# tauzn-clock/mpsfm

Hardware: AMD Instinct MI355X
Metric: BA residual-evals/sec (LM iterations/sec alongside), 200 imgs / 150k pts prior-BA (higher is better)
Workload: dtype f64; 1 GPU; C3: 200 cameras, 150000 landmarks per rank, 749145 reprojection + 674306 log-depth blocks per rank, SoftL1/Cauchy, Ceres-default LM; parallelism=single GPU, residual_blocks_total=1423451

## Files before the change

### include/mpsfm_hip_debug.h

```cpp
#ifndef MPSFM_HIP_DEBUG_H
#define MPSFM_HIP_DEBUG_H

#include "mpsfm_hip.h"

#ifdef __cplusplus
extern "C" {
#endif

typedef struct mpsfm_plan_handle mpsfm_plan_handle;

void mpsfm_debug_set(int f);
int mpsfm_debug_set_chol_trace(long long* dev_buf);
int mpsfm_debug_panel_factor(const double* dx, int waves, double* out, int* ok);

mpsfm_plan_handle* mpsfm_debug_plan_create(const uint8_t* adj, int32_t n, int32_t depth, int32_t pinv_max_tiles, int32_t inv_rows);
void mpsfm_debug_plan_destroy(mpsfm_plan_handle* h);
int64_t mpsfm_debug_plan_get(const mpsfm_plan_handle* h, int32_t what, int32_t* out, int64_t cap);

int64_t mpsfm_debug_host_cache(int64_t bytes, int32_t count);
int64_t mpsfm_debug_run_parts(int32_t nparts, int32_t reps);
int mpsfm_debug_graph_union(const uint8_t* adj, int32_t world, int32_t n, uint8_t* out);

int mpsfm_debug_pt_handoff(mpsfm_ba_handle* h);
int mpsfm_debug_direct_front(mpsfm_ba_handle* h);
int mpsfm_debug_direct_assemble(mpsfm_ba_handle* h, double radius, double* A_parent, double* A_direct, double* damp, uint8_t* live, int64_t info[4]);
int mpsfm_debug_dense_solve_given(mpsfm_ba_handle* h, const double* S, const double* rhs, int32_t n, int32_t* failed);
int mpsfm_debug_read_trace(mpsfm_ba_handle* h, long long* out, int64_t count);
int64_t mpsfm_debug_table(mpsfm_ba_handle* h, int32_t which, void* out, int64_t cap);
int64_t mpsfm_debug_host_build(const mpsfm_ba_problem* P, int32_t which, void* out, int64_t cap);
int mpsfm_debug_local_clocks(mpsfm_ba_handle* h, int64_t out[12]);
int mpsfm_debug_local_skew(int32_t chunk, int32_t phase_mask, int64_t ticks);
typedef struct mpsfm_debug_lm_ctl {
  double radius, decrease_factor, x_norm, cur_cost, fixed_cost, initial_cost;
  double last_x_cost, last_cand, last_rel, last_step_norm, last_mcc;
  int32_t term, iter, invalid_run, check_gradient, accepted, n_success, n_unsuccess, n_cost_evals, n_jac_evals, last_chol_fail, trace_len, pad_;
  double trace_cost[MPSFM_MAX_TRACE], trace_radius[MPSFM_MAX_TRACE];
  uint8_t trace_accepted[MPSFM_MAX_TRACE];
} mpsfm_debug_lm_ctl;
typedef struct mpsfm_debug_lm_opts {
  double function_tolerance, gradient_tolerance, parameter_tolerance, min_relative_decrease, max_radius, min_radius;
  int32_t max_iterations, max_invalid_steps;
} mpsfm_debug_lm_opts;
int mpsfm_debug_lm_decide(int32_t form, const mpsfm_debug_lm_ctl* ctl_in, const mpsfm_debug_lm_opts* opts, double* scal, const double* redsc, const double* part,
// ... 8 lines not shown
```

### mpsfm_amd/abi.py

```python

from __future__ import annotations

import ctypes as C
import os

MAX_TRACE = 64
INT_MAX_IRLS = 16

TERMINATION_NAMES = {
    0: "function_tolerance",
    1: "gradient_tolerance",
    2: "parameter_tolerance",
    3: "max_iterations",
    4: "min_radius",
    5: "invalid_steps",
    6: "no_variables",
}

ALLREDUCE_FN = C.CFUNCTYPE(C.c_int, C.c_void_p, C.POINTER(C.c_double), C.c_int64, C.c_int, C.c_void_p)


class CProblem(C.Structure):
    _c_name_ = "mpsfm_ba_problem"
    _fields_ = [
# ... 428 lines not shown
    "mpsfm_debug_set": (None, [C.c_int]),
    "mpsfm_debug_set_chol_trace": (C.c_int, [P]),
    "mpsfm_debug_panel_factor": (C.c_int, [P, C.c_int, P, C.POINTER(C.c_int)]),
    "mpsfm_debug_plan_create": (P, [P, I32, I32, I32, I32]),
    "mpsfm_debug_plan_destroy": (None, [P]),
    "mpsfm_debug_plan_get": (I64, [P, I32, P, I64]),
    "mpsfm_debug_host_cache": (I64, [I64, I32]),
    "mpsfm_debug_run_parts": (I64, [I32, I32]),
    "mpsfm_debug_graph_union": (C.c_int, [P, I32, I32, P]),
    "mpsfm_debug_pt_handoff": (C.c_int, [P]),
    "mpsfm_debug_direct_front": (C.c_int, [P]),
    "mpsfm_debug_direct_assemble": (C.c_int, [P, C.c_double, P, P, P, P, P]),
    "mpsfm_debug_dense_solve_given": (C.c_int, [P, P, P, I32, C.POINTER(I32)]),
    "mpsfm_debug_read_trace": (C.c_int, [P, P, I64]),
    "mpsfm_debug_table": (I64, [P, I32, P, I64]),
    "mpsfm_debug_host_build": (I64, [P, I32, P, I64]),
    "mpsfm_debug_local_clocks": (C.c_int, [P, P]),
    "mpsfm_debug_local_skew": (C.c_int, [I32, I32, I64]),
    "mpsfm_debug_lm_decide": (C.c_int, [I32, P, P, P, P, P, P, I64, I32, P, P, P]),
    "mpsfm_debug_resources": (C.c_int, [I32, P]),
}


LIB_PATH = os.path.join(os.path.dirname(os.path.abspath(__file__)), "libmpsfm_hip.so")

_lib = None


class MpsfmHipError(RuntimeError):
    def __init__(self, code: int, msg: str):
# ... 21 lines not shown
```

### mpsfm_amd/build.py

```python

from __future__ import annotations

import os
import subprocess
import sys

HERE = os.path.dirname(os.path.abspath(__file__))
CSRC = os.path.join(HERE, "csrc")
LIB = os.path.join(HERE, "libmpsfm_hip.so")
SOURCES = ["ba_kernels.hip", "sweep_dense.hip", "local_lm.hip", "build_dev.hip", "build_host.hip", "dense_chol.hip", "dev_resources.hip", "ba_comm.hip", "ba_build.hip", "ba_solver.hip", "ba_debug.hip", "tri_kernels.hip", "int_kernels.hip", "prior_kernels.hip", "triangulator.hip", "chol_plan.hip", "depth_consistency.hip", "abs_pose.hip", "rel_pose.hip", "two_view.hip", "two_view_batch.hip", "registration.hip", "dense_matches.hip", "descriptor_matches.hip", "descriptor_matches_batch.hip", "retrieval.hip", "reciprocal_matches.hip", "warp_matches.hip", "mono_priors.hip", "corr_graph.hip"]
HEADERS = ["common.h", "dev_resources.h", "ba_launch.h", "ba_handle.h", "devbuild.h", "build_host.h", "host_parts.h", "sweep_common.h", "sweep_dense_body.h", "sweep_update_body.h", "dense_tile.h", "lm_decide.h", "local_lm.h", "tri_math.h", "bilinear_sample.h", "abs_pose_math.h", "rel_pose_math.h", "rel_pose_problem.h", "two_view_math.h", "two_view_problem.h", "chol_plan.h", "call_scope.h", "lo_ransac.h", "point_grid.h", "resize_taps.h", "sim_tile.h", "sim_top2.h", "sim_topk.h", os.path.join("..", "..", "include", "mpsfm_hip.h"),
           os.path.join("..", "..", "include", "mpsfm_hip_debug.h")]


def _hipcc() -> str:
    for c in (os.environ.get("HIPCC"), "/opt/rocm/bin/hipcc", "hipcc"):
        if c and (os.path.isabs(c) and os.path.exists(c) or not os.path.isabs(c)):
            return c
    return "hipcc"


FLAGS_STAMP = os.path.join(HERE, "build", "extra_flags.txt")


def _flags_changed() -> bool:
# ... 52 lines not shown
```

### mpsfm_amd/capi.py

```python

from __future__ import annotations

import ctypes as C

import numpy as np

from .abi import (
    ALLREDUCE_FN, LIB_PATH, SIGNATURES, CAbsPoseOptions, CAbsPoseResult, CCorrGraphInfo, CDcImage, CDebugLmCtl, CDebugLmOpts, CDcSummary, CDepthGather, CDepthPriorConf,
    CDepthPriorOutput, CDepthPriorProblem, CInitCandidates, CInitPair, CIntProblem, CIntSummary, CMatchBatchReport, CMatchInfo, CMatchOptions, CNmsInfo,
    CNormalPriorConf, CNormalPriorOutput, CNormalPriorProblem, COptions, CPriorSummary, CProblem, CRansacOptions, CRecipInfo,
    CRecipOptions, CRegImage, CRelPoseOptions, CRetrievalInfo, CRetrievalOptions, CRelPoseResult, CState, CSummary, CTracks, CTriCandidates, CTwoViewBatchReport, CTwoViewLeg, CTwoViewOptions,
    CTwoViewResult, CWarpInfo, CWarpOptions, MpsfmHipError, lib,
)
from .problem import BAProblem, Tracks

EXPORTS = list(SIGNATURES)
_MATCH_DESC_ARGS = SIGNATURES["mpsfm_match_descriptors"][1]
_MATCH_MAP_ARGS = SIGNATURES["mpsfm_match_map_descriptors"][1]
_SIMPLE_NMS_ARGS = SIGNATURES["mpsfm_simple_nms"][1]
_KPIDS_ARGS = SIGNATURES["mpsfm_kpids_to_matches0"][1]
_WARP_ARGS = SIGNATURES["mpsfm_warp_matches"][1]


def _check(rc: int):
# ... 117 lines not shown

    def pt_handoff(self) -> bool:
        return bool(lib().mpsfm_debug_pt_handoff(self._h))

    def direct_front(self) -> bool:
        return bool(lib().mpsfm_debug_direct_front(self._h))

    def direct_assemble(self, radius: float = 1e4) -> dict:
        nt = self.dense_plan()["tile_columns"]
        ntiles = (nt + 1) * (nt + 2) // 2
        ap, ad = np.zeros((ntiles, 32, 32)), np.zeros((ntiles, 32, 32))
        damp, live, info = np.zeros(32 * nt), np.zeros(ntiles, np.uint8), np.zeros(4, np.int64)
        _check(lib().mpsfm_debug_direct_assemble(self._h, float(radius), ap.ctypes.data, ad.ctypes.data, damp.ctypes.data, live.ctypes.data, info.ctypes.data))
        assert int(info[0]) == nt
        return dict(parent=ap, direct=ad, damp=damp, live=live.astype(bool), nt=nt, n=int(info[1]), n_live=int(info[2]), unzeroed=int(info[3]))

    def sweep_once(self, radius: float = 1e4) -> float:
        ms = C.c_float(0)
        _check(lib().mpsfm_ba_sweep_once(self._h, radius, C.byref(ms)))
        return ms.value

    def sweep_parts(self) -> dict:
        ms, info = (C.c_float * 3)(), (C.c_int64 * 4)()
        _check(lib().mpsfm_ba_sweep_parts(self._h, ms, info))
        return dict(dense_ms=ms[0], reduce_ms=ms[1], general_ms=ms[2], dense_chunks=int(info[0]), general_chunks=int(info[1]),
                    long_tracks=int(info[2]), reduce_parts=int(info[3]))

    def dense_solve_once(self) -> float:
        ms = C.c_float(0)
        _check(lib().mpsfm_ba_dense_solve_once(self._h, C.byref(ms)))
# ... 1108 lines not shown
```

### mpsfm_amd/csrc/ba_debug.hip

```cpp
#include <algorithm>
#include <atomic>
#include <cstring>
#include <limits>
#include <vector>

#include "../../include/mpsfm_hip_debug.h"
#include "ba_handle.h"

using namespace mpsfm;

static void dense_plan_numbers(int ncv, int nt, const CholPlan& P, const DenseOverlap& ov, const LevelPlanDev& lp, double* work, int64_t sblk, int64_t v[10]) {
  const bool level = dense_level(&ov, &lp);
  const bool pinv = level && dense_pinv(work, nt, &ov, &lp) != nullptr;
  const int64_t w[10] = {ncv, nt, level ? P.nlevels : nt, P.nd_depth, pinv ? 1 : 0, (int64_t)P.items.size(), P.products, P.roles, sblk,
                         pinv ? 1 : (level ? P.nlevels : (nt + 3) / 4 + 1)};
  for (int i = 0; i < 10; ++i) v[i] = w[i];
}

extern "C" int64_t mpsfm_debug_host_cache(int64_t bytes, int32_t count) {
  std::vector<mpsfm::HostBuf<uint8_t>> first((size_t)count), second((size_t)count);
  std::vector<const void*> seen;
  for (auto& b : first) { b.alloc((size_t)bytes); b[0] = 1; b[(size_t)bytes - 1] = 2; seen.push_back(b.data()); }
  first.clear();
  int64_t reused = 0;
// ... 152 lines not shown
  MPSFM_TRY(hipMemcpyAsync(A_direct, h->d_A, sizeof(double) * img.size(), hipMemcpyDeviceToHost, s));
  MPSFM_TRY(hipMemcpyAsync(pinv.data(), a.zero_P, sizeof(double) * pinv.size(), hipMemcpyDeviceToHost, s));
  MPSFM_TRY(hipMemcpyAsync(y.data(), h->d_yc, sizeof(double) * (size_t)h->n_user, hipMemcpyDeviceToHost, s));
  MPSFM_TRY(hipMemcpyAsync(dcol.data(), h->d_diag_col, sizeof(double) * dcol.size(), hipMemcpyDeviceToHost, s));
  MPSFM_TRY(hipStreamSynchronize(s));
  MPSFM_TRY(hipGetLastError());
  h->last_radius = radius;
  const int32_t* slot_of_col = h->plan.slot_of_col.empty() ? nullptr : h->plan.slot_of_col.data();
  for (int g = 0; g < nt * 32; ++g)
    damp[g] = vec_index(slot_of_col, g, h->n) < 0 ? -1.0 : std::min(std::max(dcol[(size_t)g], h->opt.min_lm_diagonal), h->opt.max_lm_diagonal) / radius;
  int64_t bad = 0;
  for (double v : pinv) bad += v == 0.0 ? 0 : 1;
  for (int i = 0; i < h->n_user; ++i) bad += y[(size_t)i] == 0.0 ? 0 : 1;
  info[0] = nt; info[1] = h->n; info[2] = (int64_t)h->plan.asm_tiles.size(); info[3] = bad;
  return 0;
}

int mpsfm_ba_sweep_once(mpsfm_ba_handle* h, double radius, float* elapsed_ms) {
  if (!h) return fail(MPSFM_EINVAL, "handle is NULL");
  MPSFM_TRY(hipSetDevice(h->device));
  if (!h->scales_ready) if (int rc = prepare_scales(h)) return rc;
  MPSFM_TRY(hipMemsetAsync(h->d_red, 0, sizeof(double) * (size_t)h->red_count, h->stream));
  SweepArgs a = sweep_args(h, radius);
  MPSFM_TRY(hipEventRecord(h->ev[0], h->stream));
  launch_track_sweep_dense(a, h->n_dense, h->stream);
  MPSFM_TRY(hipEventRecord(h->ev[1], h->stream));
  launch_reduce_slabs(h->d_red_dests, h->n_red_dests, h->d_red_srcs, h->d_slab, h->d_Sblk, h->d_gc, h->d_wv, h->d_diagU, nullptr, h->stream);
  MPSFM_TRY(hipEventRecord(h->ev[2], h->stream));
  a.chunk0 = h->n_dense;
  launch_track_sweep(a, h->nchunks - h->n_dense, false, h->stream);
// ... 46 lines not shown
    case 20: src = h->d_red_srcs; bytes = 4 * h->n_red_srcs; break;
    case 21: src = h->cam_slot_h.data(); bytes = 4 * (int64_t)h->cam_slot_h.size(); host = true; break;
    case 23: src = h->d_blk_desc; bytes = 4 * h->n_blk_desc; break;
    case 24: src = h->d_blk_ent_start; bytes = 4 * h->n_blk_ent_start; break;
    case 25: src = h->d_ents; bytes = 4 * h->n_ents; break;
    case 26: src = h->d_part; bytes = 32 * (int64_t)h->nchunks; break;
    case 22: { static uint8_t flag; flag = h->built_on_device ? 1 : 0; src = &flag; bytes = 1; host = true; break; }
    case 27: src = h->d_lhdr; bytes = (int64_t)sizeof(LongHdr) * h->nlong; break;
    case 28: src = h->spat.sky_index.data(); bytes = 4 * (int64_t)h->spat.sky_index.size(); host = true; break;
    case 29: src = h->spat.sky_first.data(); bytes = 4 * (int64_t)h->spat.sky_first.size(); host = true; break;
    case 30: src = h->spat.sky_start.data(); bytes = 8 * (int64_t)h->spat.sky_start.size(); host = true; break;
    case 31: src = h->d_cmask; bytes = 48 * (int64_t)h->nc; break;
    case 32: src = h->d_cam_of_slot; bytes = 4 * (int64_t)std::max(h->ncv, 1); break;
    case 33: { static thread_local int64_t info[10]; if (int rc = mpsfm_ba_dense_plan(h, info)) return rc; src = info; bytes = 80; host = true; break; }
    case 34: src = h->last_launches; bytes = (int64_t)sizeof(h->last_launches); host = true; break;
    default: return fail(MPSFM_EINVAL, "unknown table");
  }
  if (!out || cap < bytes) return bytes;
  if (bytes == 0) return 0;
  if (host) { std::memcpy(out, src, (size_t)bytes); return bytes; }
  if (hipSetDevice(h->device) != hipSuccess) return fail(MPSFM_EHIP, "hipSetDevice failed");
  if (hipMemcpyAsync(out, src, (size_t)bytes, hipMemcpyDeviceToHost, h->stream) != hipSuccess) return fail(MPSFM_EHIP, "copy failed");
  if (hipStreamSynchronize(h->stream) != hipSuccess) return fail(MPSFM_EHIP, "sync failed");
  return bytes;
}

int64_t mpsfm_debug_host_build(const mpsfm_ba_problem* P, int32_t which, void* out, int64_t cap) {
  if (int rc = check_problem(P)) return rc;
  BuildOptions opt = BuildOptions::from_environment();
  TableBuild B;
// ... 177 lines not shown
```

### mpsfm_amd/csrc/ba_handle.h

```cpp
#pragma once
#include <cstdint>
#include <memory>
#include <vector>

#include "ba_launch.h"
#include "build_host.h"
#include "common.h"
#include "dev_resources.h"
#include "devbuild.h"

struct mpsfm_ba_handle {
  int device = 0;
  mpsfm::DeviceBlocks own;
  hipStream_t stream = nullptr;
  void* comm = nullptr;
  mpsfm::DenseOverlap ov;
  mpsfm::SPattern spat;
  mpsfm::BlockSky sky{nullptr, nullptr, nullptr, 0};
  mpsfm::CholPlan plan;
  mpsfm::LevelPlanDev lp;
  std::vector<int32_t> nat_slot;
  int n_user = 0;
  mpsfm_ba_options opt{};
  mpsfm::LossParams loss{};
// ... 73 lines not shown
int build_tables(const mpsfm_ba_problem* P, BuildOptions& opt, const SumExchange& exchange, bool sharded, int verbose, const Lap& lap, DeviceStages* dev,
                 TableBuild& out);
void level_plan_flags(const CholPlan& PL, LevelPlanDev& D);

int create_impl(const mpsfm_ba_problem* P, const mpsfm_ba_state* st, const mpsfm_ba_options* o, mpsfm_ba_handle** out);
int upload_state(mpsfm_ba_handle* h, const mpsfm_ba_state* st, bool as_initial);
void free_handle(mpsfm_ba_handle* h);

int comm_init_rank(mpsfm_ba_handle* h);
void comm_destroy(void* comm);
int allreduce_host(mpsfm_ba_handle* h, double* buf, int64_t count);
int allreduce_dev(mpsfm_ba_handle* h, double* buf, int64_t count);

SweepArgs sweep_args(mpsfm_ba_handle* h, double radius, const LmCtl* ctl = nullptr);
int prepare_scales(mpsfm_ba_handle* h);
int run_track_sweep(mpsfm_ba_handle* h, double radius, const LmCtl* ctl = nullptr, bool in_loop = false, bool adopt = false, bool handoff = false,
                    bool direct = false);
void run_assemble(mpsfm_ba_handle* h, double radius, const LmCtl* ctl = nullptr);
int run_dense(mpsfm_ba_handle* h, double radius, const LmCtl* ctl = nullptr, bool direct = false);
bool direct_front(mpsfm_ba_handle* h);
DirectAsm direct_asm(const mpsfm_ba_handle* h);
void direct_zero_args(mpsfm_ba_handle* h, SweepArgs& a);
bool chol_entry_list();

struct LocalSkew { int32_t chunk = 0, mask = 0; int64_t ticks = 0; };
extern LocalSkew g_local_skew;

}
```

### mpsfm_amd/csrc/ba_launch.h

```cpp
#pragma once
#include "common.h"
#include "local_lm.h"

namespace mpsfm {
enum LaunchFamily {
  kLfTrackSweep,
  kLfReduceSlabs,
  kLfAssemble,
  kLfCholLevel,
  kLfDenseRest,
  kLfUpdateSweep,
  kLfDecide,
  kLfScales,
  kLfOther,
  kLfCount
};
extern thread_local int64_t g_launches[kLfCount];
inline void count_launch(LaunchFamily f, int n = 1) { g_launches[f] += n; }

void launch_track_sweep(const SweepArgs&, int nchunks, bool diag_only, hipStream_t);
void launch_update_sweep(const SweepArgs&, int nchunks, hipStream_t, const CamUpdArgs* cu = nullptr);
void launch_track_sweep_dense(const SweepArgs&, int nchunks, hipStream_t);
void launch_reduce_slabs(const RedDest* dests, int ndest, const int32_t* srcs, const double* slab, double* Sblk, double* gc, double* wv, double* diagU,
                         const LmCtl* ctl, hipStream_t, const DirectAsm* direct = nullptr);
// ... 10 lines not shown
constexpr int kReduceThreads = 1024;
void launch_lm_decide(LmCtl* ctl, double* scal, const LmOpts& o, LmCtl* host_copy, hipStream_t, const double* redsc = nullptr);
void launch_zero(double* p, int64_t n, const LmCtl* ctl, hipStream_t);
void launch_lm_reduce_decide(const double* part, const double* part2, int64_t rows, LmCtl* ctl, double* scal, const LmOpts& o, LmCtl* host_copy, hipStream_t);
void launch_lm_prologue(const LmCtl* ctl, double* red, int64_t nred, int nc, int64_t np, double* q, double* t, double* camtab, double* pts, const double* q2,
                        const double* t2, const double* camtab2, const double* pts2, hipStream_t);
void launch_lm_accept(const LmCtl* ctl, int nc, int64_t np, double* q, double* t, double* camtab, double* pts, const double* q2, const double* t2,
                      const double* camtab2, const double* pts2, hipStream_t);
void launch_pts_sqnorm(int64_t np, const uint16_t* pt_kv, const double* pts, double* part, int nblocks, hipStream_t);
void launch_gmax_to_slot(double* redsc, int rank, hipStream_t);
void launch_lm_pack(const double* scal, double* sums, hipStream_t);
void launch_lm_init(LmCtl* ctl, const double* scal, const double* sums, hipStream_t);
void launch_permute_pts(int64_t np, const int32_t* perm, const double* src, double* dst, bool scatter, hipStream_t);
void launch_gmax_from_slots(const double* redsc, double* scal, hipStream_t);

extern int g_dbg_flags;
void launch_assemble(const AssembleArgs&, hipStream_t);
void launch_dense_solve(double* A, double* work, int nt, int n, double* y, int* fail, hipStream_t, DenseOverlap* ov, const LevelPlanDev* lp,
                        const LmCtl* ctl = nullptr, const DampArgs* damp = nullptr);
bool dense_level(const DenseOverlap* ov, const LevelPlanDev* lp);
int dense_plain_max_tiles();
int dense_inv_rows();
size_t dense_work_doubles(int nt);
double* dense_pinv(double* work, int nt, const DenseOverlap* ov, const LevelPlanDev* lp);

int local_lm_max_chunks(int device);
int launch_local_lm(const LocalArgs& a, hipStream_t s);

}
```

### mpsfm_amd/csrc/ba_solver.hip

```cpp
#include <algorithm>
#include <chrono>
#include <cstdio>
#include <cstdlib>
#include <cstring>
#include <vector>

#include "ba_handle.h"

namespace mpsfm {

LocalSkew g_local_skew;

SweepArgs sweep_args(mpsfm_ba_handle* h, double radius, const LmCtl* ctl) {
  SweepArgs a{};
  a.ctl = ctl;
  a.chunks = h->d_chunks; a.chunk_cams = h->d_chunk_cams; a.rec_cam = h->rt.rec_cam; a.rec_meta = h->rt.rec_meta;
  a.rec_xy = h->rt.rec_xy; a.rec_d = h->rt.rec_d; a.rec_m = h->rt.rec_m; a.rec_a = h->rt.rec_a;
  a.pt_rec_start = h->rt.pt_rec_start; a.pt_kv = h->rt.pt_kv; a.blk_desc = h->d_blk_desc; a.blk_ent_start = h->d_blk_ent_start; a.ents = h->d_ents;
  a.camtab = h->d_camtab; a.pts = h->d_pts; a.ps = h->d_ps; a.loss = h->loss;
  a.radius = radius; a.min_diag = h->opt.min_lm_diagonal; a.max_diag = h->opt.max_lm_diagonal; a.ncv = h->ncv; a.dbg = (g_dbg_flags >> 8) & 0xff;
  a.lhdr = h->d_lhdr; a.nlong = h->nlong; a.nchunks = h->nchunks; a.cam_slot = h->d_cam_slot; a.wl = h->d_wl;
  a.sky = h->sky;
  a.Sblk = h->d_Sblk; a.gc = h->d_gc; a.wv = h->d_wv; a.diagU = h->d_diagU; a.part = h->d_part; a.diagV = h->d_diagV;
  a.yc = h->d_yc; a.camtab2 = h->d_camtab2; a.pts2 = h->d_pts2; a.part2 = h->d_part2;
// ... 136 lines not shown
  sum->num_iterations = last.iter;
  sum->num_successful_steps = last.n_success;
  sum->num_unsuccessful_steps = last.n_unsuccess;
  sum->termination = last.term;
  sum->final_radius = last.radius;
  sum->trace_len = last.trace_len;
  for (int i = 0; i < last.trace_len; ++i) { sum->trace_cost[i] = last.trace_cost[i]; sum->trace_radius[i] = last.trace_radius[i]; sum->trace_accepted[i] = last.trace_accepted[i]; }
  return 0;
}

constexpr int kLocalRefused = 1;
constexpr double kSplitMinFront = 40e-6;
bool chol_entry_list() { const char* e = std::getenv("MPSFM_CHOL_ENTRY"); return e && std::strcmp(e, "list") == 0; }
static bool pt_handoff_enabled() { const char* e = std::getenv("MPSFM_PT_HANDOFF"); return !(e && std::atoi(e) == 0); }

static int solve_local(mpsfm_ba_handle* h, mpsfm_ba_summary* sum) {
  hipStream_t s = h->stream;
  const mpsfm_ba_options& o = h->opt;
  launch_cam_scales(h->nc, h->d_cam_slot, h->d_cmask, h->d_diagU, 0, h->d_cs, s);
  launch_build_camtab(h->nc, h->d_q, h->d_t, h->d_intr, h->d_intr_idx, h->d_cs, h->d_camtab, s);
  double* fixed_parts = h->d_scal + 12;
  MPSFM_TRY(hipMemsetAsync(h->d_scal, 0, sizeof(double) * U_COUNT, s));
  launch_fixed_cost(h, fixed_parts);
  if (int rc = prepare_scales(h)) return rc;
  h->h_ctl[0] = initial_ctl(o);
  MPSFM_TRY(hipMemcpyAsync(h->d_ctl, &h->h_ctl[0], sizeof(LmCtl), hipMemcpyHostToDevice, s));
  MPSFM_TRY(hipMemsetAsync(h->d_local_acc, 0, sizeof(double) * 2 * kLocalAccDoubles, s));
  MPSFM_TRY(hipMemsetAsync(h->d_local_sync, 0, sizeof(int64_t) * 16, s));
  LocalArgs la{};
  la.A = sweep_args(h, 0.0, nullptr);
  if (pt_handoff_enabled()) la.A.pt_fac = h->d_pt_fac;
  la.ctl = h->d_ctl;
  la.o = lm_opts_of(o);
  la.log = o.verbose > 0 ? h->d_local_log : nullptr;
  la.acc[0] = h->d_local_acc; la.acc[1] = h->d_local_acc + kLocalAccDoubles;
  la.part[0] = h->d_part; la.part[1] = h->d_part + (size_t)h->nchunks * 4;
  la.bar = reinterpret_cast<int32_t*>(h->d_local_sync); la.clk = reinterpret_cast<long long*>(h->d_local_sync + 1);
  la.ncv = h->ncv; la.nc = h->nc; la.nchunks = h->nchunks;
  la.q = h->d_q; la.t = h->d_t; la.camtab = h->d_camtab; la.pts = h->d_pts; la.cs = h->d_cs; la.fixed_parts = fixed_parts;
  la.skew_chunk = g_local_skew.chunk; la.skew_mask = g_local_skew.ticks > 0 ? g_local_skew.mask : 0; la.skew_ticks = g_local_skew.ticks;
  if (launch_local_lm(la, s) != (int)hipSuccess) {
    (void)hipGetLastError();
    MPSFM_TRY(hipStreamSynchronize(s));
// ... 29 lines not shown
  MPSFM_TRY(hipStreamSynchronize(s));
  const auto t_begin = clk::now();
  sum->num_residual_blocks = (int64_t)h->nblocks_global;
  sum->reduced_dim = h->n_user;
  std::fill(g_launches, g_launches + kLfCount, (int64_t)0);
  auto finish = [&](int rc) {
    std::copy(g_launches, g_launches + kLfCount, h->last_launches);
    sum->time_total_s = std::chrono::duration<double>(clk::now() - t_begin).count();
    return rc;
  };
  if (h->local_ok) {
    const int rc = solve_local(h, sum);
    if (rc != kLocalRefused) return finish(rc);
  }

  launch_cam_scales(h->nc, h->d_cam_slot, h->d_cmask, h->d_diagU, 0, h->d_cs, s);
  launch_build_camtab(h->nc, h->d_q, h->d_t, h->d_intr, h->d_intr_idx, h->d_cs, h->d_camtab, s);
  if (h->n == 0 && h->nvarpts_global == 0.0) {
    double fx[3], c3[3];
    if (int rc = cost_of_records(h, true, fx)) return rc;
    double fixed = fx[0] + fx[1];
    if (int rc = allreduce_host(h, &fixed, 1)) return rc;
    sum->fixed_cost = fixed;
    if (int rc = cost_of_records(h, false, c3)) return rc;
    double c = c3[0] + c3[1];
    if (int rc = allreduce_host(h, &c, 1)) return rc;
    sum->initial_cost = sum->final_cost = c + fixed;
    sum->termination = MPSFM_TERM_NO_VARIABLES;
    return finish(0);
  }
  MPSFM_TRY(hipMemsetAsync(h->d_scal, 0, sizeof(double) * U_COUNT, s));
  launch_fixed_cost(h, h->d_scal + 12);
  if (int rc = prepare_scales(h)) return rc;
  if (h->np > 0) MPSFM_TRY(hipMemcpyAsync(h->d_pts2, h->d_pts, sizeof(double) * 3 * h->np, hipMemcpyDeviceToDevice, s));
  MPSFM_TRY(hipMemsetAsync(h->d_yc, 0, sizeof(double) * (size_t)std::max(h->n_user, 1), s));
  MPSFM_TRY(hipMemsetAsync(h->d_gc, 0, sizeof(double) * (size_t)std::max(h->n_user, 1), s));
  launch_cam_update(h->nc, h->d_cam_slot, h->d_q, h->d_t, h->d_cs, h->d_yc, h->d_gc, h->d_q2, h->d_t2, h->d_scal, s);
  const int nb = (int)std::min<int64_t>(1024, std::max<int64_t>(1, (h->np + kThreads - 1) / kThreads));
  launch_pts_sqnorm(h->np, h->rt.pt_kv, h->d_pts, h->d_costpart, nb, s);
  launch_reduce_cols(h->d_costpart, nb, 1, 1, 0u, h->d_scal + U_XN_SQ_PTS, s);

  h->h_ctl[0] = initial_ctl(o);
  MPSFM_TRY(hipMemcpyAsync(h->d_ctl, &h->h_ctl[0], sizeof(LmCtl), hipMemcpyHostToDevice, s));
  double* sums = nullptr;
  if (sharded(h)) {
    sums = h->d_costpart;
    launch_lm_pack(h->d_scal, sums, s);
    if (int rc = allreduce_dev(h, sums, 3)) return rc;
  }
  launch_lm_init(h->d_ctl, h->d_scal, sums, s);
  const LmOpts lo = lm_opts_of(o);
  const LmCtl* ctl = h->d_ctl;
  const double no_radius = 0.0;
  const bool fuse_prologue = [] { const char* e = std::getenv("MPSFM_FUSE_PROLOGUE"); return !(e && std::atoi(e) == 0); }();
  const bool fuse_cam = [] { const char* e = std::getenv("MPSFM_FUSE_CAM"); return !(e && std::atoi(e) == 0); }();
  const bool pt_handoff = pt_handoff_enabled() && h->d_pt_fac != nullptr;
  h->ov.entry_list = chol_entry_list();
  const bool fused_prologue = fuse_prologue && h->nlong == 0 && h->n_dense > 0 && h->n_dense == h->nchunks;
  const bool direct = fused_prologue && direct_front(h);
  auto enqueue_front = [&](int it) -> int {
    hipEvent_t* ev = (it & 1) ? h->ev2 : h->ev;
    MPSFM_TRY(hipEventRecord(ev[0], s));
    if (!fused_prologue)
      launch_lm_prologue(h->d_ctl, h->d_red, h->red_count, h->nc, h->np, h->d_q, h->d_t, h->d_camtab, h->d_pts, h->d_q2, h->d_t2, h->d_camtab2, h->d_pts2, s);
    if (int rc = run_track_sweep(h, no_radius, ctl, true, fused_prologue, pt_handoff, direct)) return rc;
// ... 187 lines not shown
```

Measured before the change: 9.990 billion residual-block evals/s.

## Fuse BA solve setup into begin, diagonal-sweep and scales kernels

Replaces the chain of small setup launches, memsets, copies and reductions that run before the LM loop (camera scales, camtab build, scale preparation, point copy and norm, camera update, control init) with three kernels. A begin kernel clears buffers and the control block, a per-chunk diagonal sweep computes the Jacobi diagonals and also copies points and partial norms, and a single-block kernel finishes the camera scales, candidates and control fields. This cuts per-solve launch and host overhead. It adds a second linearization path that has to stay consistent with prepare_scales, and an env var keeps the old launch path available.

```diff
diff --git a/include/mpsfm_hip_debug.h b/include/mpsfm_hip_debug.h
--- a/include/mpsfm_hip_debug.h
+++ b/include/mpsfm_hip_debug.h
@@ -27,6 +27,7 @@
 int mpsfm_debug_dense_solve_given(mpsfm_ba_handle* h, const double* S, const double* rhs, int32_t n, int32_t* failed);
 int mpsfm_debug_read_trace(mpsfm_ba_handle* h, long long* out, int64_t count);
 int64_t mpsfm_debug_table(mpsfm_ba_handle* h, int32_t which, void* out, int64_t cap);
+int mpsfm_debug_solve_setup(mpsfm_ba_handle* h, int32_t local);
 int64_t mpsfm_debug_host_build(const mpsfm_ba_problem* P, int32_t which, void* out, int64_t cap);
 int mpsfm_debug_local_clocks(mpsfm_ba_handle* h, int64_t out[12]);
 int mpsfm_debug_local_skew(int32_t chunk, int32_t phase_mask, int64_t ticks);
diff --git a/mpsfm_amd/abi.py b/mpsfm_amd/abi.py
--- a/mpsfm_amd/abi.py
+++ b/mpsfm_amd/abi.py
@@ -466,6 +466,7 @@
     "mpsfm_debug_dense_solve_given": (C.c_int, [P, P, P, I32, C.POINTER(I32)]),
     "mpsfm_debug_read_trace": (C.c_int, [P, P, I64]),
     "mpsfm_debug_table": (I64, [P, I32, P, I64]),
+    "mpsfm_debug_solve_setup": (C.c_int, [P, I32]),
     "mpsfm_debug_host_build": (I64, [P, I32, P, I64]),
     "mpsfm_debug_local_clocks": (C.c_int, [P, P]),
     "mpsfm_debug_local_skew": (C.c_int, [I32, I32, I64]),
diff --git a/mpsfm_amd/build.py b/mpsfm_amd/build.py
--- a/mpsfm_amd/build.py
+++ b/mpsfm_amd/build.py
@@ -8,7 +8,7 @@
 HERE = os.path.dirname(os.path.abspath(__file__))
 CSRC = os.path.join(HERE, "csrc")
 LIB = os.path.join(HERE, "libmpsfm_hip.so")
-SOURCES = ["ba_kernels.hip", "sweep_dense.hip", "local_lm.hip", "build_dev.hip", "build_host.hip", "dense_chol.hip", "dev_resources.hip", "ba_comm.hip", "ba_build.hip", "ba_solver.hip", "ba_debug.hip", "tri_kernels.hip", "int_kernels.hip", "prior_kernels.hip", "triangulator.hip", "chol_plan.hip", "depth_consistency.hip", "abs_pose.hip", "rel_pose.hip", "two_view.hip", "two_view_batch.hip", "registration.hip", "dense_matches.hip", "descriptor_matches.hip", "descriptor_matches_batch.hip", "retrieval.hip", "reciprocal_matches.hip", "warp_matches.hip", "mono_priors.hip", "corr_graph.hip"]
+SOURCES = ["ba_kernels.hip", "sweep_dense.hip", "solve_setup.hip", "local_lm.hip", "build_dev.hip", "build_host.hip", "dense_chol.hip", "dev_resources.hip", "ba_comm.hip", "ba_build.hip", "ba_solver.hip", "ba_debug.hip", "tri_kernels.hip", "int_kernels.hip", "prior_kernels.hip", "triangulator.hip", "chol_plan.hip", "depth_consistency.hip", "abs_pose.hip", "rel_pose.hip", "two_view.hip", "two_view_batch.hip", "registration.hip", "dense_matches.hip", "descriptor_matches.hip", "descriptor_matches_batch.hip", "retrieval.hip", "reciprocal_matches.hip", "warp_matches.hip", "mono_priors.hip", "corr_graph.hip"]
 HEADERS = ["common.h", "dev_resources.h", "ba_launch.h", "ba_handle.h", "devbuild.h", "build_host.h", "host_parts.h", "sweep_common.h", "sweep_dense_body.h", "sweep_update_body.h", "dense_tile.h", "lm_decide.h", "local_lm.h", "tri_math.h", "bilinear_sample.h", "abs_pose_math.h", "rel_pose_math.h", "rel_pose_problem.h", "two_view_math.h", "two_view_problem.h", "chol_plan.h", "call_scope.h", "lo_ransac.h", "point_grid.h", "resize_taps.h", "sim_tile.h", "sim_top2.h", "sim_topk.h", os.path.join("..", "..", "include", "mpsfm_hip.h"),
            os.path.join("..", "..", "include", "mpsfm_hip_debug.h")]
 
diff --git a/mpsfm_amd/capi.py b/mpsfm_amd/capi.py
--- a/mpsfm_amd/capi.py
+++ b/mpsfm_amd/capi.py
@@ -155,6 +155,20 @@
         _check(lib().mpsfm_debug_direct_assemble(self._h, float(radius), ap.ctypes.data, ad.ctypes.data, damp.ctypes.data, live.ctypes.data, info.ctypes.data))
         assert int(info[0]) == nt
         return dict(parent=ap, direct=ad, damp=damp, live=live.astype(bool), nt=nt, n=int(info[1]), n_live=int(info[2]), unzeroed=int(info[3]))
+
+    def solve_setup(self, local: int = -1) -> dict:
+        rc = lib().mpsfm_debug_solve_setup(self._h, int(local))
+        if rc < 0:
+            _check(rc)
+        out = {"fused": bool(rc)}
+        for code, name, width in ((35, "cs", 6), (36, "ps", 3), (37, "camtab", 24), (38, "q2", 4), (39, "t2", 3), (40, "pts2", 3), (41, "x_norm", 0),
+                                  (42, "fixed_cost", 0)):
+            n = int(lib().mpsfm_debug_table(self._h, code, None, 0))
+            assert n >= 0 and n % 8 == 0, (code, n)
+            v = np.zeros(n // 8)
+            assert int(lib().mpsfm_debug_table(self._h, code, v.ctypes.data, n)) == n
+            out[name] = v.reshape(-1, width) if width else float(v[0])
+        return out
 
     def sweep_once(self, radius: float = 1e4) -> float:
         ms = C.c_float(0)
diff --git a/mpsfm_amd/csrc/ba_debug.hip b/mpsfm_amd/csrc/ba_debug.hip
--- a/mpsfm_amd/csrc/ba_debug.hip
+++ b/mpsfm_amd/csrc/ba_debug.hip
@@ -190,6 +190,17 @@
   for (int i = 0; i < h->n_user; ++i) bad += y[(size_t)i] == 0.0 ? 0 : 1;
   info[0] = nt; info[1] = h->n; info[2] = (int64_t)h->plan.asm_tiles.size(); info[3] = bad;
   return 0;
+}
+
+int mpsfm_debug_solve_setup(mpsfm_ba_handle* h, int32_t local) {
+  if (!h) return fail(MPSFM_EINVAL, "handle is NULL");
+  if (local > 0 && !h->local_ok) return fail(MPSFM_EUNSUPPORTED, "the handle does not take the single-launch solver");
+  MPSFM_TRY(hipSetDevice(h->device));
+  const bool fused = setup_fused(h);
+  if (int rc = setup_solve(h, local < 0 ? h->local_ok : local > 0)) return rc < 0 ? rc : -rc;
+  MPSFM_TRY(hipStreamSynchronize(h->stream));
+  MPSFM_TRY(hipGetLastError());
+  return fused ? 1 : 0;
 }
 
 int mpsfm_ba_sweep_once(mpsfm_ba_handle* h, double radius, float* elapsed_ms) {
@@ -266,6 +277,14 @@
     case 32: src = h->d_cam_of_slot; bytes = 4 * (int64_t)std::max(h->ncv, 1); break;
     case 33: { static thread_local int64_t info[10]; if (int rc = mpsfm_ba_dense_plan(h, info)) return rc; src = info; bytes = 80; host = true; break; }
     case 34: src = h->last_launches; bytes = (int64_t)sizeof(h->last_launches); host = true; break;
+    case 35: src = h->d_cs; bytes = 48 * (int64_t)h->nc; break;
+    case 36: src = h->d_ps; bytes = 24 * h->np; break;
+    case 37: src = h->d_camtab; bytes = 8 * (int64_t)kCamRec * h->nc; break;
+    case 38: src = h->d_q2; bytes = 32 * (int64_t)h->nc; break;
+    case 39: src = h->d_t2; bytes = 24 * (int64_t)h->nc; break;
+    case 40: src = h->d_pts2; bytes = 24 * h->np; break;
+    case 41: src = &h->d_ctl->x_norm; bytes = 8; break;
+    case 42: src = &h->d_ctl->fixed_cost; bytes = 8; break;
     default: return fail(MPSFM_EINVAL, "unknown table");
   }
   if (!out || cap < bytes) return bytes;
diff --git a/mpsfm_amd/csrc/ba_handle.h b/mpsfm_amd/csrc/ba_handle.h
--- a/mpsfm_amd/csrc/ba_handle.h
+++ b/mpsfm_amd/csrc/ba_handle.h
@@ -111,6 +111,8 @@
 
 SweepArgs sweep_args(mpsfm_ba_handle* h, double radius, const LmCtl* ctl = nullptr);
 int prepare_scales(mpsfm_ba_handle* h);
+int setup_solve(mpsfm_ba_handle* h, bool local);
+bool setup_fused(const mpsfm_ba_handle* h);
 int run_track_sweep(mpsfm_ba_handle* h, double radius, const LmCtl* ctl = nullptr, bool in_loop = false, bool adopt = false, bool handoff = false,
                     bool direct = false);
 void run_assemble(mpsfm_ba_handle* h, double radius, const LmCtl* ctl = nullptr);
diff --git a/mpsfm_amd/csrc/ba_launch.h b/mpsfm_amd/csrc/ba_launch.h
--- a/mpsfm_amd/csrc/ba_launch.h
+++ b/mpsfm_amd/csrc/ba_launch.h
@@ -48,6 +48,27 @@
 void launch_permute_pts(int64_t np, const int32_t* perm, const double* src, double* dst, bool scatter, hipStream_t);
 void launch_gmax_from_slots(const double* redsc, double* scal, hipStream_t);
 
+struct SetupArgs {
+  int32_t nc, n_user;
+  const int32_t* cam_slot; const double* cmask; const double* q; const double* t; const double* intr; const int32_t* intr_idx;
+  double* cs; double* camtab;
+  double* diagU; double* yc; double* gc; double* scal;
+  LmCtl* ctl; double radius0;
+  double* local_acc; int64_t n_local_acc;
+  int64_t* local_sync;
+  double* q2; double* t2;
+  const double* norm_part; int32_t n_norm_part;
+  int32_t init_ctl;
+};
+struct DiagArgs {
+  double* ps;
+  int64_t np;
+  double* norm_part;
+};
+void launch_solve_begin(const SetupArgs&, hipStream_t);
+void launch_diag_sweep(const SweepArgs&, const DiagArgs&, int nchunks, hipStream_t);
+void launch_solve_scales(const SetupArgs&, hipStream_t);
+
 extern int g_dbg_flags;
 void launch_assemble(const AssembleArgs&, hipStream_t);
 void launch_dense_solve(double* A, double* work, int nt, int n, double* y, int* fail, hipStream_t, DenseOverlap* ov, const LevelPlanDev* lp,
diff --git a/mpsfm_amd/csrc/ba_solver.hip b/mpsfm_amd/csrc/ba_solver.hip
--- a/mpsfm_amd/csrc/ba_solver.hip
+++ b/mpsfm_amd/csrc/ba_solver.hip
@@ -174,19 +174,76 @@
 bool chol_entry_list() { const char* e = std::getenv("MPSFM_CHOL_ENTRY"); return e && std::strcmp(e, "list") == 0; }
 static bool pt_handoff_enabled() { const char* e = std::getenv("MPSFM_PT_HANDOFF"); return !(e && std::atoi(e) == 0); }
 
+static int setup_launches(mpsfm_ba_handle* h, bool local) {
+  hipStream_t s = h->stream;
+  launch_cam_scales(h->nc, h->d_cam_slot, h->d_cmask, h->d_diagU, 0, h->d_cs, s);
+  launch_build_camtab(h->nc, h->d_q, h->d_t, h->d_intr, h->d_intr_idx, h->d_cs, h->d_camtab, s);
+  MPSFM_TRY(hipMemsetAsync(h->d_scal, 0, sizeof(double) * U_COUNT, s));
+  launch_fixed_cost(h, h->d_scal + 12);
+  if (int rc = prepare_scales(h)) return rc;
+  h->h_ctl[0] = initial_ctl(h->opt);
+  if (local) {
+    MPSFM_TRY(hipMemcpyAsync(h->d_ctl, &h->h_ctl[0], sizeof(LmCtl), hipMemcpyHostToDevice, s));
+    MPSFM_TRY(hipMemsetAsync(h->d_local_acc, 0, sizeof(double) * 2 * kLocalAccDoubles, s));
+    MPSFM_TRY(hipMemsetAsync(h->d_local_sync, 0, sizeof(int64_t) * 16, s));
+    return 0;
+  }
+  if (h->np > 0) MPSFM_TRY(hipMemcpyAsync(h->d_pts2, h->d_pts, sizeof(double) * 3 * h->np, hipMemcpyDeviceToDevice, s));
+  MPSFM_TRY(hipMemsetAsync(h->d_yc, 0, sizeof(double) * (size_t)std::max(h->n_user, 1), s));
+  MPSFM_TRY(hipMemsetAsync(h->d_gc, 0, sizeof(double) * (size_t)std::max(h->n_user, 1), s));
+  launch_cam_update(h->nc, h->d_cam_slot, h->d_q, h->d_t, h->d_cs, h->d_yc, h->d_gc, h->d_q2, h->d_t2, h->d_scal, s);
+  const int nb = (int)std::min<int64_t>(1024, std::max<int64_t>(1, (h->np + kThreads - 1) / kThreads));
+  launch_pts_sqnorm(h->np, h->rt.pt_kv, h->d_pts, h->d_costpart, nb, s);
+  launch_reduce_cols(h->d_costpart, nb, 1, 1, 0u, h->d_scal + U_XN_SQ_PTS, s);
+  MPSFM_TRY(hipMemcpyAsync(h->d_ctl, &h->h_ctl[0], sizeof(LmCtl), hipMemcpyHostToDevice, s));
+  double* sums = nullptr;
+  if (sharded(h)) {
+    sums = h->d_costpart;
+    launch_lm_pack(h->d_scal, sums, s);
+    if (int rc = allreduce_dev(h, sums, 3)) return rc;
+  }
+  launch_lm_init(h->d_ctl, h->d_scal, sums, s);
+  return 0;
+}
+bool setup_fused(const mpsfm_ba_handle* h) {
+  const char* e = std::getenv("MPSFM_SOLVE_SETUP");
+  if (e && std::strcmp(e, "launches") == 0) return false;
+  return h->opt.jacobi_scaling != 0 && h->nlong == 0 && h->nchunks > 0 && h->nc > 0;
+}
+int setup_solve(mpsfm_ba_handle* h, bool local) {
+  if (!setup_fused(h)) return setup_launches(h, local);
+  hipStream_t s = h->stream;
+  SetupArgs P{};
+  P.nc = h->nc; P.n_user = h->n_user;
+  P.cam_slot = h->d_cam_slot; P.cmask = h->d_cmask; P.q = h->d_q; P.t = h->d_t; P.intr = h->d_intr; P.intr_idx = h->d_intr_idx;
+  P.cs = h->d_cs; P.camtab = h->d_camtab;
+  P.diagU = h->d_diagU; P.yc = h->d_yc; P.gc = h->d_gc; P.scal = h->d_scal;
+  P.ctl = h->d_ctl; P.radius0 = h->opt.initial_trust_region_radius;
+  if (local) { P.local_acc = h->d_local_acc; P.n_local_acc = 2 * (int64_t)kLocalAccDoubles; P.local_sync = h->d_local_sync; }
+  else { P.q2 = h->d_q2; P.t2 = h->d_t2; P.norm_part = h->d_part2; P.n_norm_part = h->nchunks; P.init_ctl = sharded(h) ? 0 : 1; }
+  launch_solve_begin(P, s);
+  launch_fixed_cost(h, h->d_scal + 12);
+  const DiagArgs D{h->d_ps, h->np, local ? nullptr : h->d_part2};
+  launch_diag_sweep(sweep_args(h, 1.0), D, h->nchunks, s);
+  if (int rc = allreduce_dev(h, h->d_diagU, h->n_user)) return rc;
+  launch_solve_scales(P, s);
+  h->h_ctl[0] = initial_ctl(h->opt);
+  if (!local && sharded(h)) {
+    double* sums = h->d_costpart;
+    launch_lm_pack(h->d_scal, sums, s);
+    if (int rc = allreduce_dev(h, sums, 3)) return rc;
+    launch_lm_init(h->d_ctl, h->d_scal, sums, s);
+  }
+  MPSFM_TRY(hipGetLastError());
+  h->scales_ready = true;
+  return 0;
+}
+
 static int solve_local(mpsfm_ba_handle* h, mpsfm_ba_summary* sum) {
   hipStream_t s = h->stream;
   const mpsfm_ba_options& o = h->opt;
-  launch_cam_scales(h->nc, h->d_cam_slot, h->d_cmask, h->d_diagU, 0, h->d_cs, s);
-  launch_build_camtab(h->nc, h->d_q, h->d_t, h->d_intr, h->d_intr_idx, h->d_cs, h->d_camtab, s);
   double* fixed_parts = h->d_scal + 12;
-  MPSFM_TRY(hipMemsetAsync(h->d_scal, 0, sizeof(double) * U_COUNT, s));
-  launch_fixed_cost(h, fixed_parts);
-  if (int rc = prepare_scales(h)) return rc;
-  h->h_ctl[0] = initial_ctl(o);
-  MPSFM_TRY(hipMemcpyAsync(h->d_ctl, &h->h_ctl[0], sizeof(LmCtl), hipMemcpyHostToDevice, s));
-  MPSFM_TRY(hipMemsetAsync(h->d_local_acc, 0, sizeof(double) * 2 * kLocalAccDoubles, s));
-  MPSFM_TRY(hipMemsetAsync(h->d_local_sync, 0, sizeof(int64_t) * 16, s));
+  if (int rc = setup_solve(h, true)) return rc;
   LocalArgs la{};
   la.A = sweep_args(h, 0.0, nullptr);
   if (pt_handoff_enabled()) la.A.pt_fac = h->d_pt_fac;
@@ -246,9 +303,9 @@
     if (rc != kLocalRefused) return finish(rc);
   }
 
-  launch_cam_scales(h->nc, h->d_cam_slot, h->d_cmask, h->d_diagU, 0, h->d_cs, s);
-  launch_build_camtab(h->nc, h->d_q, h->d_t, h->d_intr, h->d_intr_idx, h->d_cs, h->d_camtab, s);
   if (h->n == 0 && h->nvarpts_global == 0.0) {
+    launch_cam_scales(h->nc, h->d_cam_slot, h->d_cmask, h->d_diagU, 0, h->d_cs, s);
+    launch_build_camtab(h->nc, h->d_q, h->d_t, h->d_intr, h->d_intr_idx, h->d_cs, h->d_camtab, s);
     double fx[3], c3[3];
     if (int rc = cost_of_records(h, true, fx)) return rc;
     double fixed = fx[0] + fx[1];
@@ -261,26 +318,8 @@
     sum->termination = MPSFM_TERM_NO_VARIABLES;
     return finish(0);
   }
-  MPSFM_TRY(hipMemsetAsync(h->d_scal, 0, sizeof(double) * U_COUNT, s));
-  launch_fixed_cost(h, h->d_scal + 12);
-  if (int rc = prepare_scales(h)) return rc;
-  if (h->np > 0) MPSFM_TRY(hipMemcpyAsync(h->d_pts2, h->d_pts, sizeof(double) * 3 * h->np, hipMemcpyDeviceToDevice, s));
-  MPSFM_TRY(hipMemsetAsync(h->d_yc, 0, sizeof(double) * (size_t)std::max(h->n_user, 1), s));
-  MPSFM_TRY(hipMemsetAsync(h->d_gc, 0, sizeof(double) * (size_t)std::max(h->n_user, 1), s));
-  launch_cam_update(h->nc, h->d_cam_slot, h->d_q, h->d_t, h->d_cs, h->d_yc, h->d_gc, h->d_q2, h->d_t2, h->d_scal, s);
-  const int nb = (int)std::min<int64_t>(1024, std::max<int64_t>(1, (h->np + kThreads - 1) / kThreads));
-  launch_pts_sqnorm(h->np, h->rt.pt_kv, h->d_pts, h->d_costpart, nb, s);
-  launch_reduce_cols(h->d_costpart, nb, 1, 1, 0u, h->d_scal + U_XN_SQ_PTS, s);
-
-  h->h_ctl[0] = initial_ctl(o);
-  MPSFM_TRY(hipMemcpyAsync(h->d_ctl, &h->h_ctl[0], sizeof(LmCtl), hipMemcpyHostToDevice, s));
-  double* sums = nullptr;
-  if (sharded(h)) {
-    sums = h->d_costpart;
-    launch_lm_pack(h->d_scal, sums, s);
-    if (int rc = allreduce_dev(h, sums, 3)) return rc;
-  }
-  launch_lm_init(h->d_ctl, h->d_scal, sums, s);
+  if (int rc = setup_solve(h, false)) return rc;
+
   const LmOpts lo = lm_opts_of(o);
   const LmCtl* ctl = h->d_ctl;
   const double no_radius = 0.0;
diff --git a/mpsfm_amd/csrc/solve_setup.hip b/mpsfm_amd/csrc/solve_setup.hip
--- /dev/null
+++ b/mpsfm_amd/csrc/solve_setup.hip
@@ -0,0 +1,191 @@
+#include "common.h"
+#include "ba_launch.h"
+#include "sweep_common.h"
+#include <algorithm>
+
+namespace mpsfm {
+
+__device__ __forceinline__ void camtab_row(const SetupArgs& P, int i, const double (&cs6)[6]) {
+  double* o = P.camtab + (size_t)i * kCamRec;
+  quat_to_R(P.q + 4 * i, o);
+  o[9] = P.t[3 * i]; o[10] = P.t[3 * i + 1]; o[11] = P.t[3 * i + 2];
+  const double* K = P.intr + 4 * P.intr_idx[i];
+  o[12] = K[0]; o[13] = K[1]; o[14] = K[2]; o[15] = K[3];
+  for (int k = 0; k < 6; ++k) { o[16 + k] = cs6[k]; P.cs[6 * i + k] = cs6[k]; }
+  o[22] = o[23] = 0.0;
+}
+
+__global__ __launch_bounds__(256) void k_solve_begin(SetupArgs P) {
+  const int64_t g0 = (int64_t)blockIdx.x * 256 + threadIdx.x, gstep = (int64_t)gridDim.x * 256;
+  for (int64_t i = g0; i < P.nc; i += gstep) {
+    const bool var = P.cam_slot[i] >= 0;
+    double cs6[6];
+#pragma unroll
+    for (int k = 0; k < 6; ++k) cs6[k] = var ? P.cmask[6 * i + k] : 0.0;
+    camtab_row(P, (int)i, cs6);
+  }
+  for (int64_t e = g0; e < P.n_user; e += gstep) { P.diagU[e] = 0.0; P.yc[e] = 0.0; P.gc[e] = 0.0; }
+  for (int64_t e = g0; e < U_COUNT; e += gstep) P.scal[e] = 0.0;
+  if (P.local_acc) {
+    for (int64_t e = g0; e < P.n_local_acc; e += gstep) P.local_acc[e] = 0.0;
+    for (int64_t e = g0; e < 16; e += gstep) P.local_sync[e] = 0;
+  }
+  if (blockIdx.x == 0) {
+    static_assert(sizeof(LmCtl) % 8 == 0, "the control block is cleared in 8-byte words");
+    unsigned long long* w = reinterpret_cast<unsigned long long*>(P.ctl);
+    for (int e = threadIdx.x; e < (int)(sizeof(LmCtl) / 8); e += 256) w[e] = 0ull;
+    __syncthreads();
+    if (threadIdx.x == 0) { P.ctl->radius = P.radius0; P.ctl->decrease_factor = 2.0; P.ctl->term = kLmRunning; P.ctl->check_gradient = 1; }
+  }
+}
+
+__device__ __forceinline__ double tree16(const double* p, bool is_max) {
+  double a[4];
+#pragma unroll
+  for (int k = 0; k < 4; ++k)
+    a[k] = is_max ? fmax(fmax(p[4 * k], p[4 * k + 1]), fmax(p[4 * k + 2], p[4 * k + 3])) : (p[4 * k] + p[4 * k + 1]) + (p[4 * k + 2] + p[4 * k + 3]);
+  return is_max ? fmax(fmax(a[0], a[1]), fmax(a[2], a[3])) : (a[0] + a[1]) + (a[2] + a[3]);
+}
+__global__ __launch_bounds__(kReduceThreads) void k_solve_scales(SetupArgs P) {
+  constexpr int kWaves = kReduceThreads / 64;
+  static_assert(kWaves == 16, "tree16 sums sixteen wave results");
+  __shared__ double s_red[4 * kWaves];
+  const double zero6[6] = {0.0, 0.0, 0.0, 0.0, 0.0, 0.0};
+  double step = 0.0, xn = 0.0, gmax = 0.0;
+  for (int i = threadIdx.x; i < P.nc; i += kReduceThreads) {
+    const int slot = P.cam_slot[i];
+    double cs6[6];
+#pragma unroll
+    for (int k = 0; k < 6; ++k) cs6[k] = slot >= 0 ? P.cmask[6 * i + k] / (1.0 + sqrt(P.diagU[(size_t)slot * 6 + k])) : 0.0;
+    camtab_row(P, i, cs6);
+    if (P.q2) {
+      const double qq[4] = {P.q[4 * i], P.q[4 * i + 1], P.q[4 * i + 2], P.q[4 * i + 3]};
+      const double tt[3] = {P.t[3 * i], P.t[3 * i + 1], P.t[3 * i + 2]};
+      double qn[4] = {qq[0], qq[1], qq[2], qq[3]}, tn[3] = {tt[0], tt[1], tt[2]};
+      if (slot >= 0) camera_candidate(qq, tt, cs6, zero6, zero6, qn, tn, step, xn, gmax);
+      for (int k = 0; k < 4; ++k) P.q2[4 * i + k] = qn[k];
+      for (int k = 0; k < 3; ++k) P.t2[3 * i + k] = tn[k];
+    }
+  }
+  if (!P.q2) return;
+  step = wave_sum(step); xn = wave_sum(xn); gmax = wave_max(gmax);
+  double xp = 0.0;
+  for (int r = threadIdx.x; r < P.n_norm_part; r += kReduceThreads) xp += P.norm_part[r];
+  xp = wave_sum(xp);
+  const int w = threadIdx.x >> 6;
+  if ((threadIdx.x & 63) == 0) { s_red[w] = step; s_red[kWaves + w] = xn; s_red[2 * kWaves + w] = gmax; s_red[3 * kWaves + w] = xp; }
+  __syncthreads();
+  if (threadIdx.x == 0) {
+    const double xn_cams = tree16(s_red + kWaves, false), xn_pts = tree16(s_red + 3 * kWaves, false);
+    P.scal[U_STEP_SQ_CAMS] = tree16(s_red, false);
+    P.scal[U_XN_SQ_CAMS] = xn_cams;
+    P.scal[U_GMAX_CAMS] = tree16(s_red + 2 * kWaves, true);
+    P.scal[U_XN_SQ_PTS] = xn_pts;
+    if (P.init_ctl) {
+      P.ctl->x_norm = sqrt(xn_pts + xn_cams);
+      P.ctl->fixed_cost = P.scal[12] + P.scal[13];
+    }
+  }
+}
+
+__global__ __launch_bounds__(kThreads, 5) void k_diag_sweep(SweepArgs A, DiagArgs D) {
+  __shared__ double s_v[kPtsMax * 3];
+  __shared__ double s_du[kTileCams * 6];
+  __shared__ double s_red[kThreads / 64];
+  const int tid = threadIdx.x;
+  const ChunkHdr H = A.chunks[blockIdx.x];
+  const int nrec = H.nrec, npt = H.npt, ncam = H.ncam;
+  const bool has_rec = tid < nrec;
+  for (int i = tid; i < npt * 3; i += kThreads) s_v[i] = 0.0;
+  if (tid < kTileCams * 6) s_du[tid] = 0.0;
+  __syncthreads();
+
+  uint32_t my_meta = 0;
+  uint16_t my_kv = 0xffff;
+  double Vd[3] = {0.0, 0.0, 0.0};
+  if (has_rec) {
+    const int rix = H.rec0 + tid;
+    const uint32_t meta = A.rec_meta[rix];
+    my_meta = meta;
+    const int cam = A.rec_cam[rix];
+    const int lcam = meta & 0xff, lpt = (meta >> 8) & 0xff;
+    const double2 xy = reinterpret_cast<const double2*>(A.rec_xy)[rix];
+    double d = 1.0, m = 0.0, a = 1.0;
+    if (meta & kRecHasDepth) { d = A.rec_d[rix]; m = A.rec_m[rix]; a = A.rec_a[rix]; }
+    const int pix = H.pt0 + lpt;
+    const double X[3] = {A.pts[3 * pix], A.pts[3 * pix + 1], A.pts[3 * pix + 2]};
+    my_kv = A.pt_kv[pix];
+    const double one = my_kv != 0xffff ? 1.0 : 0.0;
+    const double psc[3] = {one, one, one};
+    RecLin L;
+    linearize_record(A.camtab + (size_t)cam * kCamRec, X, psc, meta, xy.x, xy.y, d, m, a, A.loss, L);
+    if (L.ok) {
+      if (one != 0.0) {
+#pragma unroll
+        for (int r = 0; r < 3; ++r) { Vd[0] += L.Jp[3 * r] * L.Jp[3 * r]; Vd[1] += L.Jp[3 * r + 1] * L.Jp[3 * r + 1]; Vd[2] += L.Jp[3 * r + 2] * L.Jp[3 * r + 2]; }
+      }
+      if (lcam != (int)kLcamConst) {
+        const int slot = lcam < kTileCams ? 0 : A.chunk_cams[H.cam0 + lcam];
+#pragma unroll
+        for (int i = 0; i < 6; ++i) {
+          const double du = L.Jc[i] * L.Jc[i] + L.Jc[6 + i] * L.Jc[6 + i] + L.Jc[12 + i] * L.Jc[12 + i];
+          if (lcam < kTileCams) atomicAdd(&s_du[lcam * 6 + i], du);
+          else atomicAdd(&A.diagU[(size_t)slot * 6 + i], du);
+        }
+      }
+    }
+  }
+  static_assert(kPtsMax <= 0xff, "0xff is no record's landmark");
+  const int my_lpt = has_rec ? (int)((my_meta >> 8) & 0xff) : 0xff;
+  seg_step<1>(my_lpt, Vd); seg_step<2>(my_lpt, Vd); seg_step<4>(my_lpt, Vd); seg_step<8>(my_lpt, Vd);
+  const int nlpt = __builtin_amdgcn_update_dpp(-1, my_lpt, 0x101, 0xf, 0xf, false);
+  if (nlpt != my_lpt && my_lpt < npt) {
+#pragma unroll
+    for (int k = 0; k < 3; ++k) if (Vd[k] != 0.0) atomicAdd(&s_v[my_lpt * 3 + k], Vd[k]);
+  }
+  __syncthreads();
+  const int prev_lpt = (__shfl_up((int)my_meta, 1, 64) >> 8) & 0xff;
+  if (has_rec && my_kv != 0xffff && ((tid & 63) == 0 || prev_lpt != my_lpt)) {
+    double* o = D.ps + (size_t)3 * (H.pt0 + my_lpt);
+#pragma unroll
+    for (int k = 0; k < 3; ++k) o[k] = 1.0 / (1.0 + sqrt(s_v[my_lpt * 3 + k]));
+  }
+  if (tid < kTileCams * 6) {
+    const int lc = tid / 6;
+    if (lc < ncam && s_du[tid] != 0.0) atomicAdd(&A.diagU[(size_t)A.chunk_cams[H.cam0 + lc] * 6 + (tid - lc * 6)], s_du[tid]);
+  }
+
+  if (D.norm_part == nullptr) return;
+  const int64_t per = (D.np + gridDim.x - 1) / gridDim.x;
+  const int64_t i0 = std::min<int64_t>(D.np, per * blockIdx.x), i1 = std::min<int64_t>(D.np, i0 + per);
+  double acc = 0.0;
+  for (int64_t e = 3 * i0 + tid; e < 3 * i1; e += kThreads) {
+    const int64_t i = e / 3;
+    const double v = A.pts[e];
+    A.pts2[e] = v;
+    if (A.pt_kv[i] == 0xffff) D.ps[e] = 0.0;
+    else acc += v * v;
+  }
+  acc = wave_sum(acc);
+  if ((tid & 63) == 0) s_red[tid >> 6] = acc;
+  __syncthreads();
+  if (tid == 0) D.norm_part[blockIdx.x] = (s_red[0] + s_red[1]) + (s_red[2] + s_red[3]);
+}
+
+void launch_solve_begin(const SetupArgs& P, hipStream_t s) {
+  const int64_t work = std::max<int64_t>(std::max<int64_t>(P.nc, P.n_user), P.local_acc ? P.n_local_acc : 0);
+  const int grid = (int)std::min<int64_t>(64, std::max<int64_t>(1, (work + 255) / 256));
+  count_launch(kLfScales);
+  hipLaunchKernelGGL(k_solve_begin, dim3(grid), dim3(256), 0, s, P);
+}
+void launch_diag_sweep(const SweepArgs& a, const DiagArgs& d, int nchunks, hipStream_t s) {
+  if (nchunks <= 0) return;
+  count_launch(kLfTrackSweep);
+  hipLaunchKernelGGL(k_diag_sweep, dim3(nchunks), dim3(kThreads), 0, s, a, d);
+}
+void launch_solve_scales(const SetupArgs& P, hipStream_t s) {
+  count_launch(kLfScales);
+  hipLaunchKernelGGL(k_solve_scales, dim3(1), dim3(kReduceThreads), 0, s, P);
+}
+
+}
```

New measurement: 10.05 billion residual-block evals/s (median of 6 runs). Within noise of the previous version (+0.6%).
